# locuslab/icnn

Measured on NVIDIA H100. Metric: inner-loop solves/sec (batch x iters), higher is better.
Workload: dtype f32 (K1 PICNN f/grad) + f64 (K2 bundle solve)

## Files before the change

icnn_b200/csrc/bundle_pc.cu:

```cuda
#include "bundle_pc_kernel.cuh"

#include <cstdio>
#include <cstdlib>

namespace icnn {

#define ICNN_PC_DECL(NAME) cudaError_t launch_pc_##NAME(const PcArgs& a, const PcConfig& c, int B, cudaStream_t st)
ICNN_PC_DECL(1x1); ICNN_PC_DECL(1x2);
ICNN_PC_DECL(1x1_scalar); ICNN_PC_DECL(1x2_scalar);
ICNN_PC_DECL(8x2);
ICNN_PC_DECL(16x2); ICNN_PC_DECL(16x4);
ICNN_PC_DECL(v3_8x4);

ICNN_PC_DECL(1x1) { return launch_pc<1, 1, true>(a, c, B, st); }
ICNN_PC_DECL(1x2) { return launch_pc<1, 2, true>(a, c, B, st); }
ICNN_PC_DECL(1x1_scalar) { return launch_pc<1, 1, false>(a, c, B, st); }
ICNN_PC_DECL(1x2_scalar) { return launch_pc<1, 2, false>(a, c, B, st); }

struct PcTestEnv { bool v3, split5; int pfa, pfb; };
static PcTestEnv pc_test_env() {
  PcTestEnv e = {true, false, 1, 8};
  if (const char* v = getenv("ICNN_PC_V3")) e.v3 = v[0] != '0';
  if (const char* v = getenv("ICNN_PC_LEGACY")) e.split5 = v[0] == '1';
  if (const char* v = getenv("ICNN_PC_PREFETCH")) {
    int pa = 0, pb = 0;
    if (sscanf(v, "%d,%d", &pa, &pb) == 2 && pa >= 0 && pa <= 8 && pb >= 0 && pb <= 64) { e.pfa = pa; e.pfb = pb; }
  }
  return e;
}

static bool pc_fits(const icnn_bundle_bufs* b, int wps, int nch, bool v3, PcConfig* out) {
  if (b->n > 128 * wps * nch) return false;
  PcConfig c;
  c.wps = wps; c.nch = nch; c.v3 = v3;
  c.npad = (b->n + 15) & ~15;
  c.vec = (b->n & 3) == 0;
  if (!c.vec && wps > 1) return false;
  c.smem = sizeof(double) * pc_group_doubles(c.npad, b->KS, wps, v3);
  if (c.smem > 227 * 1024) return false;
  if (v3) {
    if (!c.vec || 2 * (c.smem + 1024) > 228 * 1024) return false;
    c.minb = 2;
  } else if (wps == 16) c.minb = 1;
  else if (wps == 1) c.minb = 2;
  else
    c.minb = (c.smem + 1024) * (24 / wps) <= 228 * 1024 ? 3 : 2;
  *out = c;
  return true;
}

static bool pick_pc(const icnn_bundle_bufs* b, bool allow_v3, PcConfig* out) {
  const int n = b->n;
  if (b->KS > 62) return false;
  if (n <= 128) return pc_fits(b, 1, 1, false, out);
  if (n <= 256) return pc_fits(b, 1, 2, false, out);
  if (n <= 1024) return false;
  if (n <= 2048) return pc_fits(b, 8, 2, false, out);
  if (n <= 4096) return (allow_v3 && pc_fits(b, 8, 4, true, out)) || pc_fits(b, 16, 2, false, out);
  return pc_fits(b, 16, 4, false, out);
}

int bundle_pc_launch(const icnn_bundle_cfg* cfg, const icnn_bundle_bufs* b, int t, cudaStream_t st) {
  const PcTestEnv env = pc_test_env();
  PcConfig c;
  if (!pick_pc(b, env.v3, &c)) return ICNN_E_UNSUPPORTED;
  PcArgs a;
  a.b = *b; a.c = *cfg; a.t = t; a.npad = c.npad;
  a.split5 = env.split5; a.pfa = env.pfa; a.pfb = env.pfb;
  cudaError_t e;
  if (c.v3) e = launch_pc_v3_8x4(a, c, b->B, st);
  else if (c.wps == 16) e = c.nch == 2 ? launch_pc_16x2(a, c, b->B, st) : launch_pc_16x4(a, c, b->B, st);
  else if (c.wps == 8) e = launch_pc_8x2(a, c, b->B, st);
  else if (c.vec) e = c.nch == 1 ? launch_pc_1x1(a, c, b->B, st) : launch_pc_1x2(a, c, b->B, st);
  else e = c.nch == 1 ? launch_pc_1x1_scalar(a, c, b->B, st) : launch_pc_1x2_scalar(a, c, b->B, st);
  if (e != cudaSuccess) {
    set_error("bundle_pc launch (wps=%d nch=%d v3=%d smem=%zu): %s", c.wps, c.nch, (int)c.v3, c.smem, cudaGetErrorString(e));
    return ICNN_E_CUDA;
  }
  return ICNN_OK;
}

}
```

icnn_b200/csrc/bundle_pc_kernel.cuh:

```cuda
#pragma once
#include "bundle_step_kernel.cuh"

namespace icnn {

struct PcArgs {
  icnn_bundle_bufs b;
  icnn_bundle_cfg c;
  int t;
  int npad;
  int pfa;
  int pfb;
  bool split5;
};

__device__ __forceinline__ void prefetch_l2(const void* p) { asm volatile("prefetch.global.L2 [%0];" ::"l"(p)); }

constexpr int PC_NKV = 18;
constexpr int PC_NKV_V3 = 12;

__host__ __device__ inline size_t pc_group_doubles(int npad, int KS, int wps, bool v3) {
  size_t d = (size_t)(v3 ? 3 : 4) * npad + (size_t)KS * (KS + 1) / 2 +
             (size_t)(v3 ? PC_NKV_V3 : PC_NKV) * KS + KS  +
             8 * wps  + 16  + 4 ;
  return (d + 1) & ~(size_t)1;
}

__device__ __forceinline__ int lidx(int r, int c) { return r * (r + 1) / 2 + c; }

__device__ __forceinline__ double chol_dot(const double* a, const double* b, int c) {
  double t0 = 0.0, t1 = 0.0, t2 = 0.0, t3 = 0.0;
  int p = 0;
  for (; p + 3 < c; p += 4) {
    t0 = fma(a[p], b[p], t0);
    t1 = fma(a[p + 1], b[p + 1], t1);
    t2 = fma(a[p + 2], b[p + 2], t2);
    t3 = fma(a[p + 3], b[p + 3], t3);
  }
  for (; p < c; ++p) t0 = fma(a[p], b[p], t0);
  return (t0 + t1) + (t2 + t3);
}
template <bool K32>
__device__ __forceinline__ bool warp_cholesky_impl(double* L, double* invd, int k, int lane) {
  bool ok = true;
  const int r0 = lane, r1 = lane + 32;
  const int o0 = lidx(r0, 0), o1 = lidx(r1, 0);
  for (int c = 0; c < k; ++c) {
    const int oc = lidx(c, 0);
    double s0 = 0.0, s1 = 0.0;
    if (r0 >= c && r0 < k) s0 = L[o0 + c] - chol_dot(L + o0, L + oc, c);
    if (!K32) { if (r1 >= c && r1 < k) s1 = L[o1 + c] - chol_dot(L + o1, L + oc, c); }
    const double piv = K32 ? __shfl_sync(0xffffffffu, s0, c) : __shfl_sync(0xffffffffu, (c < 32) ? s0 : s1, c & 31);
    if (!(piv > 0.0) || !isfinite(piv)) { ok = false; break; }
    const double inv = rsqrt(piv);
    if (r0 > c && r0 < k) L[o0 + c] = s0 * inv;
    if (!K32) { if (r1 > c && r1 < k) L[o1 + c] = s1 * inv; }
    if (lane == 0) { L[oc + c] = piv * inv; invd[c] = inv; }
    __syncwarp();
  }
  __syncwarp();
  return ok;
}
__device__ inline bool warp_cholesky_p(double* L, double* invd, int k, int lane) {
  return k <= 32 ? warp_cholesky_impl<true>(L, invd, k, lane) : warp_cholesky_impl<false>(L, invd, k, lane);
}

template <int NR, bool K32>
__device__ __forceinline__ void warp_chol_solve_impl(const double* L, const double* invd, int k, double (&b0)[NR],
                                                     double (&b1)[NR], int lane) {
  const int r0 = lane, r1 = lane + 32;
  const int o0 = lidx(r0, 0), o1 = lidx(r1, 0);
  for (int i = 0; i < k; ++i) {
    const double di = invd[i];
    const double l0 = (r0 > i && r0 < k) ? L[o0 + i] : 0.0;
    const double l1 = (!K32 && r1 > i && r1 < k) ? L[o1 + i] : 0.0;
#pragma unroll
    for (int q = 0; q < NR; ++q) {
      const double xi = (K32 ? __shfl_sync(0xffffffffu, b0[q], i) : __shfl_sync(0xffffffffu, (i < 32) ? b0[q] : b1[q], i & 31)) * di;
      b0[q] = (r0 == i) ? xi : fma(-l0, xi, b0[q]);
      if (!K32) b1[q] = (r1 == i) ? xi : fma(-l1, xi, b1[q]);
    }
  }
  for (int i = k - 1; i >= 0; --i) {
    const double di = invd[i];
    const int oi = lidx(i, 0);
    const double l0 = (r0 < i) ? L[oi + r0] : 0.0;
    const double l1 = (!K32 && r1 < i) ? L[oi + r1] : 0.0;
#pragma unroll
    for (int q = 0; q < NR; ++q) {
      const double xi = (K32 ? __shfl_sync(0xffffffffu, b0[q], i) : __shfl_sync(0xffffffffu, (i < 32) ? b0[q] : b1[q], i & 31)) * di;
      b0[q] = (r0 == i) ? xi : fma(-l0, xi, b0[q]);
      if (!K32) b1[q] = (r1 == i) ? xi : fma(-l1, xi, b1[q]);
    }
  }
}
template <int NR>
__device__ inline void warp_chol_solve_p(const double* L, const double* invd, int k, double (&b0)[NR],
                                         double (&b1)[NR], int lane) {
  if (k <= 32) warp_chol_solve_impl<NR, true>(L, invd, k, b0, b1, lane);
  else warp_chol_solve_impl<NR, false>(L, invd, k, b0, b1, lane);
}

__device__ __forceinline__ double step2(double v0, double d0, bool ok0, double v1, double d1, bool ok1) {
  double a = 1e300;
  bool any = false;
  if (ok0 && d0 < 0.0) { a = -v0 / d0; any = true; }
  if (ok1 && d1 < 0.0) { a = fmin(a, -v1 / d1); any = true; }
  a = Grp<1>::wmin(a);
  any = __any_sync(0xffffffffu, any);
  return any ? a : 1.0;
}

template <int WPS>
struct PcRed {
  double* red;
  int par;
  template <class G>
  __device__ __forceinline__ double sum(const G& g, double v) {
    v = Grp<WPS>::wsum(v);
    if (WPS == 1) { __syncwarp(); return v; }
    double* r = red + par * 4 * WPS;
    par ^= 1;
    if (g.lane == 0) r[g.warp] = v;
    g.sync();
    double a = 0.0;
#pragma unroll
    for (int w = 0; w < WPS; ++w) a += r[w];
    return a;
  }
  template <class G>
  __device__ __forceinline__ void min2(const G& g, double& a, double& b) {
    a = Grp<WPS>::wmin(a);
    b = Grp<WPS>::wmin(b);
    if (WPS == 1) { __syncwarp(); return; }
    double* r = red + par * 4 * WPS;
    par ^= 1;
    if (g.lane == 0) { r[g.warp] = a; r[WPS + g.warp] = b; }
    g.sync();
    double ra = r[0], rb = r[WPS];
#pragma unroll
    for (int w = 1; w < WPS; ++w) { ra = fmin(ra, r[w]); rb = fmin(rb, r[WPS + w]); }
    a = ra; b = rb;
  }
};

__device__ __forceinline__ double dweight(double y) { return fma(-y, y, y); }

template <int WPS, int NA, int NB, bool TRI, bool PSEUDO, bool VEC, class G>
__device__ __forceinline__ void gram_sweep_pc(const G& g, const float* const* rowp, int k, int n, const double* yv,
                                              const double* rv, double* Lp, double* qk, double* wk, double* scratch,
                                              int scap, int a0, int b0, int pfd = 0) {
  constexpr int NT = TRI ? NA * (NA + 1) / 2 : NA * NB;
  constexpr int NL = TRI ? NB : NA + NB;
  double acc[NT][2];
#pragma unroll
  for (int t = 0; t < NT; ++t) acc[t][0] = acc[t][1] = 0.0;
  const int r = g.lane >> 2, q = g.lane & 3;
  const float* rp[NL];
  bool rok[NL];
#pragma unroll
  for (int b = 0; b < NL; ++b) {
    const int blk = TRI ? (b0 + b) : (b < NA ? a0 + b : b0 + (b - NA));
    const int row = blk * 8 + r - 2;
    rok[b] = row >= 0 && row < k;
    rp[b] = rowp[rok[b] ? row : 0] + 4 * q;
  }
  const bool ps = PSEUDO && r < 2;
  const double* yq = yv + 4 * q;
  const double* rq = rv + 4 * q;
  const int ngrp = (n + 15) >> 4;
  constexpr int NG = (NT <= 6) ? 2 : 1;
#pragma unroll 1
  for (int gi = g.warp; gi < ngrp; gi += NG * WPS) {
    float4 v[NG][NL];
#pragma unroll
    for (int u = 0; u < NG; ++u) {
      const int gu = gi + u * WPS;
      const int off = gu * 16;
      const int col = off + 4 * q;
      const bool gv = (u == 0) || gu < ngrp;
#pragma unroll
      for (int b = 0; b < NL; ++b) {
        v[u][b] = make_float4(0.f, 0.f, 0.f, 0.f);
        if (VEC) {
          if (gv && rok[b] && col < n) v[u][b] = *reinterpret_cast<const float4*>(rp[b] + off);
        } else if (gv && rok[b]) {
          const float* p = rp[b] + off;
          if (col < n) v[u][b].x = p[0];
          if (col + 1 < n) v[u][b].y = p[1];
          if (col + 2 < n) v[u][b].z = p[2];
          if (col + 3 < n) v[u][b].w = p[3];
        }
      }
    }
    if (pfd > 0) {
#pragma unroll
      for (int u = 0; u < NG; ++u) {
        const int col = (gi + (pfd * NG + u) * WPS) * 16 + 4 * q;
        if (col < n) {
#pragma unroll
          for (int b = 0; b < NL; ++b) if (rok[b]) prefetch_l2(rp[b] + (col - 4 * q));
        }
      }
    }
#pragma unroll
    for (int u = 0; u < NG; ++u) {
      const int gu = gi + u * WPS;
      if (u > 0 && gu >= ngrp) break;
      const int off = gu * 16;
      const double2 ya = *reinterpret_cast<const double2*>(yq + off);
      const double2 yb = *reinterpret_cast<const double2*>(yq + off + 2);
      double dd[4] = {dweight(ya.x), dweight(ya.y), dweight(yb.x), dweight(yb.y)};
      double pa[4] = {0.0, 0.0, 0.0, 0.0};
      if (PSEUDO && ps) {
        if (r == 0) {
          const double2 ra = *reinterpret_cast<const double2*>(rq + off);
          const double2 rb = *reinterpret_cast<const double2*>(rq + off + 2);
          pa[0] = dd[0] * ra.x; pa[1] = dd[1] * ra.y; pa[2] = dd[2] * rb.x; pa[3] = dd[3] * rb.y;
        } else {
          pa[0] = ya.x; pa[1] = ya.y; pa[2] = yb.x; pa[3] = yb.y;
        }
      }
#pragma unroll
      for (int s = 0; s < 4; ++s) {
        double f[NL];
#pragma unroll
        for (int b = 0; b < NL; ++b)
          f[b] = (double)((s == 0) ? v[u][b].x : (s == 1) ? v[u][b].y : (s == 2) ? v[u][b].z : v[u][b].w);
        int t = 0;
#pragma unroll
        for (int i = 0; i < NA; ++i) {
          const double af = (PSEUDO && i == 0) ? fma(f[0], dd[s], pa[s]) : f[i] * dd[s];
#pragma unroll
          for (int j = TRI ? i : 0; j < NB; ++j) { dmma884(acc[t][0], acc[t][1], af, f[TRI ? j : NA + j]); ++t; }
        }
      }
    }
  }
  if (WPS > 1) {
    constexpr int SLAB = NT * 64;
    const int cap = scap / SLAB;
    g.sync();
    if (cap >= 1) {
      int active = WPS;
      while (active > 1) {
        const int m = ::min(cap, active >> 1);
        if (g.warp >= active - m && g.warp < active) {
          double* sl = scratch + (size_t)(g.warp - (active - m)) * SLAB + g.lane;
#pragma unroll
          for (int t = 0; t < NT; ++t) { sl[(2 * t) * 32] = acc[t][0]; sl[(2 * t + 1) * 32] = acc[t][1]; }
        }
        g.sync();
        if (g.warp >= active - 2 * m && g.warp < active - m) {
          const double* sl = scratch + (size_t)(g.warp - (active - 2 * m)) * SLAB + g.lane;
#pragma unroll
          for (int t = 0; t < NT; ++t) { acc[t][0] += sl[(2 * t) * 32]; acc[t][1] += sl[(2 * t + 1) * 32]; }
        }
        active -= m;
        if (active > 1) g.sync();
      }
    } else {
      for (int wi = 1; wi < WPS; ++wi) {
        if (g.warp == wi) {
          int t = 0;
#pragma unroll
          for (int i = 0; i < NA; ++i)
#pragma unroll
            for (int j = TRI ? i : 0; j < NB; ++j) {
#pragma unroll
              for (int h = 0; h < 2; ++h) {
                const int ii = (a0 + i) * 8 + r, jj = (b0 + j) * 8 + 2 * q + h;
                if (jj >= 2 && jj < k + 2) {
                  if (ii < 2) { if (PSEUDO && i == 0) { double* d = (ii == 0 ? qk : wk) + (jj - 2); *d = (wi == 1 ? 0.0 : *d) + acc[t][h]; } }
                  else if (ii < k + 2 && (!(TRI && i == j) || jj >= ii)) { double* d = Lp + lidx(jj - 2, ii - 2); *d = (wi == 1 ? 0.0 : *d) + acc[t][h]; }
                }
              }
              ++t;
            }
        }
        g.sync();
      }
    }
  }
  if (g.warp == 0) {
    const bool addin = (WPS > 1) && (scap / (NT * 64) < 1);
    int t = 0;
#pragma unroll
    for (int i = 0; i < NA; ++i)
#pragma unroll
      for (int j = TRI ? i : 0; j < NB; ++j) {
#pragma unroll
        for (int h = 0; h < 2; ++h) {
          const int ii = (a0 + i) * 8 + r, jj = (b0 + j) * 8 + 2 * q + h;
          if (jj >= 2 && jj < k + 2) {
            if (ii < 2) {
              if (PSEUDO && i == 0) { double* d = (ii == 0 ? qk : wk) + (jj - 2); *d = (addin ? *d : 0.0) + acc[t][h]; }
            } else if (ii < k + 2 && (!(TRI && i == j) || jj >= ii)) {
              double* d = Lp + lidx(jj - 2, ii - 2);
              *d = (addin ? *d : 0.0) + acc[t][h];
            }
          }
        }
        ++t;
      }
    __syncwarp();
  }
}

template <int WPS, int NB, bool VEC, class G>
__device__ __forceinline__ void gram_rect_pair_pc(const G& g, const float* const* rowp, int k, int n, const double* yv,
                                                  const double* rv, double* Lp, double* qk, double* wk, double* sx, int scap,
                                                  int pfd) {
  gram_sweep_pc<WPS, 2, NB, false, true, VEC>(g, rowp, k, n, yv, rv, Lp, qk, wk, sx, scap, 0, 4, pfd);
  gram_sweep_pc<WPS, 2, NB, false, false, VEC>(g, rowp, k, n, yv, rv, Lp, qk, wk, sx, scap, 2, 4, pfd);
}

template <int WPS, bool VEC, bool ONE5, class G>
__device__ __forceinline__ void gram_pass_pc(const G& g, const float* const* rowp, int k, int n, const double* yv,
                                             const double* rv, double* Lp, double* qk, double* wk, double* sx, int scap,
                                             bool split5, int pfd) {
  const int rb = (k + 2 + 7) >> 3;
  if (rb == 1) gram_sweep_pc<WPS, 1, 1, true, true, VEC>(g, rowp, k, n, yv, rv, Lp, qk, wk, sx, scap, 0, 0, pfd);
  else if (rb == 2) gram_sweep_pc<WPS, 2, 2, true, true, VEC>(g, rowp, k, n, yv, rv, Lp, qk, wk, sx, scap, 0, 0, pfd);
  else if (rb == 3) gram_sweep_pc<WPS, 3, 3, true, true, VEC>(g, rowp, k, n, yv, rv, Lp, qk, wk, sx, scap, 0, 0, pfd);
  else if (ONE5 && rb == 5 && !split5) {
    if constexpr (ONE5) gram_sweep_pc<WPS, 5, 5, true, true, VEC>(g, rowp, k, n, yv, rv, Lp, qk, wk, sx, scap, 0, 0, pfd);
  } else {
    gram_sweep_pc<WPS, 4, 4, true, true, VEC>(g, rowp, k, n, yv, rv, Lp, qk, wk, sx, scap, 0, 0, pfd);
    if (rb > 4) {
      const int r2 = rb - 4;
      if (r2 == 1) { gram_sweep_pc<WPS, 1, 1, true, false, VEC>(g, rowp, k, n, yv, rv, Lp, qk, wk, sx, scap, 4, 4, pfd); gram_rect_pair_pc<WPS, 1, VEC>(g, rowp, k, n, yv, rv, Lp, qk, wk, sx, scap, pfd); }
      else if (r2 == 2) { gram_sweep_pc<WPS, 2, 2, true, false, VEC>(g, rowp, k, n, yv, rv, Lp, qk, wk, sx, scap, 4, 4, pfd); gram_rect_pair_pc<WPS, 2, VEC>(g, rowp, k, n, yv, rv, Lp, qk, wk, sx, scap, pfd); }
      else if (r2 == 3) { gram_sweep_pc<WPS, 3, 3, true, false, VEC>(g, rowp, k, n, yv, rv, Lp, qk, wk, sx, scap, 4, 4, pfd); gram_rect_pair_pc<WPS, 3, VEC>(g, rowp, k, n, yv, rv, Lp, qk, wk, sx, scap, pfd); }
      else { gram_sweep_pc<WPS, 4, 4, true, false, VEC>(g, rowp, k, n, yv, rv, Lp, qk, wk, sx, scap, 4, 4, pfd); gram_rect_pair_pc<WPS, 4, VEC>(g, rowp, k, n, yv, rv, Lp, qk, wk, sx, scap, pfd); }
    }
  }
}

template <int T, bool VEC>
__device__ __forceinline__ int pc_col(int cb, int tid, int c) { return VEC ? cb + 4 * tid + c : cb + tid + c * T; }

template <int T, int NR, bool VEC, int UNR = 4>
__device__ __forceinline__ void col_dots_pc(const float* const* rowp, int k, int n, int cb, int tid,
                                            const double* const (&w)[NR], double (&acc)[NR][4], int pfr = 0) {
#pragma unroll
  for (int q = 0; q < NR; ++q)
#pragma unroll
    for (int c = 0; c < 4; ++c) acc[q][c] = 0.0;
  const bool in0 = VEC ? (cb + 4 * tid < n) : (cb + tid < n);
  const bool full = VEC ? in0 : (cb + tid + 3 * T < n);
#pragma unroll UNR
  for (int j = 0; j < k; ++j) {
    const float* p = rowp[j];
    float v[4] = {0.f, 0.f, 0.f, 0.f};
    if (VEC && pfr > 0 && in0) {
      const int jp = j + pfr;
      if (jp < k) prefetch_l2(rowp[jp] + cb + 4 * tid);
      else if (jp - k < k && cb + 4 * T + 4 * tid < n) prefetch_l2(rowp[jp - k] + cb + 4 * T + 4 * tid);
    }
    if (VEC) {
      if (in0) { const float4 x = *reinterpret_cast<const float4*>(p + cb + 4 * tid); v[0] = x.x; v[1] = x.y; v[2] = x.z; v[3] = x.w; }
    } else {
#pragma unroll
      for (int c = 0; c < 4; ++c) if (full || cb + tid + c * T < n) v[c] = p[cb + tid + c * T];
    }
#pragma unroll
    for (int q = 0; q < NR; ++q) {
      const double wq = w[q][j];
#pragma unroll
      for (int c = 0; c < 4; ++c) acc[q][c] = fma((double)v[c], wq, acc[q][c]);
    }
  }
}

__device__ __forceinline__ void ratio_min(double& nm, double& dn, double a, double b) {
  if (a * dn < nm * b) { nm = a; dn = b; }
}

struct PcKxk {
  double* Lp; double* invd; const double* zc; const double* scur; const double* wk; const double* hk; const double* qk;
  double* dza; double* dzp; double* dzq; double* dsa; double* sc; int* isc;
};
template <bool K32>
__device__ __forceinline__ void pc_kxk_stage(const PcKxk& io, int k, int lane, double pr) {
  double* Lp = io.Lp;
  const int j0 = lane, j1 = lane + 32;
  const bool v0 = j0 < k, v1ok = !K32 && j1 < k;
  const double tt = io.sc[0];
  const double z0 = v0 ? io.zc[j0] : 0.0, z1 = v1ok ? io.zc[j1] : 0.0;
  const double s0 = v0 ? io.scur[j0] : 0.0, s1 = v1ok ? io.scur[j1] : 0.0;
  const double rd0 = v0 ? ((io.wk[j0] + io.hk[j0]) - tt) + s0 : 0.0;
  const double rd1 = v1ok ? ((io.wk[j1] + io.hk[j1]) - tt) + s1 : 0.0;
  const double zs = Grp<1>::wsum(z0 + z1);
  const double dr = Grp<1>::wsum(fma(rd0, rd0, rd1 * rd1));
  const double rt = 1.0 - zs;
  const bool conv = (sqrt(pr + rt * rt) < 1e-8 && sqrt(dr) < 1e-8);
  if (conv) {
    if (lane == 0) io.isc[2] = 1;
  } else {
    if (v0) Lp[lidx(j0, j0)] += s0 / z0;
    if (v1ok) Lp[lidx(j1, j1)] += s1 / z1;
    __syncwarp();
    const bool ok = warp_cholesky_impl<K32>(Lp, io.invd, k, lane);
    if (!ok) { if (lane == 0) io.isc[3] = 1; }
    else {
      const double mu = Grp<1>::wsum(fma(s0, z0, s1 * z1)) / k;
      const double ra0 = v0 ? rd0 - io.qk[j0] - s0 : 0.0, ra1 = v1ok ? rd1 - io.qk[j1] - s1 : 0.0;
      const double rp0 = v0 ? mu / z0 : 0.0, rp1 = v1ok ? mu / z1 : 0.0;
      double b0[3] = {v0 ? 1.0 : 0.0, ra0, rp0}, b1[3] = {v1ok ? 1.0 : 0.0, ra1, rp1};
      warp_chol_solve_impl<3, K32>(Lp, io.invd, k, b0, b1, lane);
      const double w1s = Grp<1>::wsum(b0[0] + b1[0]);
      const double dta = (Grp<1>::wsum(fma(ra0, b0[0], ra1 * b1[0])) - rt) / w1s;
      const double dtp = Grp<1>::wsum(fma(rp0, b0[0], rp1 * b1[0])) / w1s;
      const double da0 = fma(-dta, b0[0], b0[1]), da1 = fma(-dta, b1[0], b1[1]);
      const double dp0 = fma(-dtp, b0[0], b0[2]), dp1 = fma(-dtp, b1[0], b1[2]);
      const double dsa0 = v0 ? -(s0 / z0) * (z0 + da0) : 0.0, dsa1 = v1ok ? -(s1 / z1) * (z1 + da1) : 0.0;
      const double rq0 = v0 ? -(dsa0 * da0) / z0 : 0.0, rq1 = v1ok ? -(dsa1 * da1) / z1 : 0.0;
      double c0[1] = {rq0}, c1[1] = {rq1};
      warp_chol_solve_impl<1, K32>(Lp, io.invd, k, c0, c1, lane);
      const double dtq = Grp<1>::wsum(fma(rq0, b0[0], rq1 * b1[0])) / w1s;
      if (v0) { io.dza[j0] = da0; io.dzp[j0] = dp0; io.dzq[j0] = fma(-dtq, b0[0], c0[0]); io.dsa[j0] = dsa0; }
      if (v1ok) { io.dza[j1] = da1; io.dzp[j1] = dp1; io.dzq[j1] = fma(-dtq, b1[0], c1[0]); io.dsa[j1] = dsa1; }
      if (lane == 0) { io.sc[1] = dta; io.sc[2] = dtp; io.sc[3] = dtq; }
    }
  }
  __syncwarp();
}

template <int WPS, int NCH, bool R80, bool VEC, bool V3>
__global__ void __launch_bounds__(WPS * 32, WPS == 16 ? 1 : (R80 ? 24 : 16) / WPS) bundle_pc_kernel(PcArgs A) {
  const icnn_bundle_bufs& b = A.b;
  const icnn_bundle_cfg& cf = A.c;
  if (b.nactive[A.t] == 0) return;
  extern __shared__ __align__(16) double smem_d[];
  constexpr int GPB = 1;
  constexpr int T = WPS * 32;
  static_assert(NCH == 1 || NCH == 2 || NCH == 4, "NCH");
  Grp<WPS> g;
  g.tid = threadIdx.x % T;
  g.lane = threadIdx.x & 31;
  g.warp = g.tid >> 5;
  g.gid = threadIdx.x / T;
  const int u = blockIdx.x * GPB + g.gid;
  if (u >= b.B) return;
  if (b.finished[u]) return;

  const int n = b.n, KS = b.KS, npad = A.npad;
  double* base = smem_d + (size_t)g.gid * pc_group_doubles(npad, KS, WPS, V3);
  double* yv = base;
  double* uv = V3 ? nullptr : yv + npad;
  double* rv = V3 ? yv + npad : uv + npad;
  double* xv = rv + npad;
  double* Lp = xv + npad;
  double* kv = Lp + (size_t)KS * (KS + 1) / 2;
#define PCKV(i) (kv + (i) * KS)
  double* hk = PCKV(0);
  double* wk = PCKV(5);
  double* qk = PCKV(6);
  double* dza = PCKV(7);
  double* dzp = PCKV(8);
  double* dzq = PCKV(9);
  double* dsa = PCKV(10);
  double* invd = PCKV(11);
  double* tk = PCKV(V3 ? 7 : 12);
  double* ek = PCKV(V3 ? 8 : 13);
  double* rk = PCKV(V3 ? 9 : 14);
  const float** rowp = reinterpret_cast<const float**>(kv + (size_t)(V3 ? PC_NKV_V3 : PC_NKV) * KS);
  PcRed<WPS> red;
  red.red = reinterpret_cast<double*>(rowp + KS);
  red.par = 0;
  g.red = red.red;
  double* sc = red.red + 8 * WPS;
  int* isc = reinterpret_cast<int*>(sc + 16);

  const int k0 = b.count[u];
  const int k = k0 + 1;
  const int* permu = b.perm + (size_t)u * KS;
  float* Gu = b.G + (size_t)u * KS * n;
  double* hu = b.h + (size_t)u * KS;
  double* lamu = b.lam + (size_t)u * KS;
  double* rsu = b.rsum + (size_t)u * KS;
  double* gramu = b.gram + (size_t)u * KS * KS;
  double* yu = b.y + (size_t)u * n;
  const int slot_new = permu[k0];

  for (int j = g.tid; j < k; j += T) rowp[j] = Gu + (size_t)permu[j] * n;
  if (g.tid == 0) {
#pragma unroll
    for (int i = 0; i < 8; ++i) isc[i] = 0;
  }
  g.sync();
  const float* gnew = rowp[k0];

  {
    double hs = 0.0, rs = 0.0, bad = 0.0, ent = 0.0;
    double* ysrow = b.ys ? b.ys + ((size_t)u * KS + slot_new) * n : nullptr;
    for (int e = g.tid; e < n; e += T) {
      const double ge = (double)gnew[e];
      const double ye = yu[e];
      hs = fma(ge, ye, hs);
      rs += ge;
      if (!isfinite(ge)) bad = 1.0;
      if (ysrow) __stcs(ysrow + e, ye);
      if (b.iter_stats) ent += neg_entropy(ye);
    }
    if (b.iter_stats) ent = g.sum(ent);
    hs = g.sum(hs);
    rs = g.sum(rs);
    bad = g.max(bad);
    const double fu = b.f64 ? b.f64[u] : (double)b.f[u];
    if (g.tid == 0) { stat_add(b.iter_stats, A.t, 0, 1.0); stat_add(b.iter_stats, A.t, 6, fu + ent); }
    if (bad > 0.0 || !isfinite(fu)) {
      if (g.tid == 0) { b.status[u] = ICNN_ST_NONFINITE; b.finished[u] = 1; b.nIters[u] = A.t - 1; stat_add(b.iter_stats, A.t, 5, 1.0); }
      return;
    }
    for (int j = g.warp; j < k; j += WPS) {
      const float* rj = rowp[j];
      double acc = 0.0;
      int diff = 0;
      for (int e = g.lane; e < n; e += 32) {
        const float a = rj[e], c = gnew[e];
        acc = fma((double)a, (double)c, acc);
        diff |= (a != c);
      }
      acc = Grp<WPS>::wsum(acc);
      diff = __any_sync(0xffffffffu, diff);
      if (g.lane == 0) { tk[j] = acc; ek[j] = diff ? 1.0 : 0.0; }
    }
    if (g.tid == 0) { hu[slot_new] = fu - hs; rsu[slot_new] = rs; sc[10] = fu - hs; sc[11] = rs; }
    g.sync();
    if (g.tid == 0) {
      int dup = 0;
      for (int j = 0; j < k0; ++j) dup |= (ek[j] == 0.0);
      isc[0] = dup;
    }
    g.sync();
  }
  bool dependent = false;
  if (k > n) dependent = true;
  else if (k0 > 0) {
    if (g.warp == 0) {
      for (int i = g.lane; i < k0; i += 32)
        for (int j = 0; j <= i; ++j) Lp[lidx(i, j)] = gramu[(size_t)permu[i] * KS + permu[j]];
      __syncwarp();
      const bool ok = warp_cholesky_p(Lp, invd, k0, g.lane);
      if (ok) {
        double b0[1] = {g.lane < k0 ? tk[g.lane] : 0.0}, b1[1] = {g.lane + 32 < k0 ? tk[g.lane + 32] : 0.0};
        warp_chol_solve_p<1>(Lp, invd, k0, b0, b1, g.lane);
        if (g.lane < k0) rk[g.lane] = b0[0];
        if (g.lane + 32 < k0) rk[g.lane + 32] = b1[0];
      }
      double md = tk[k0];
      for (int j = g.lane; j < k0; j += 32) md = fmax(md, gramu[(size_t)permu[j] * KS + permu[j]]);
      md = Grp<1>::wmax(md);
      if (g.lane == 0) { isc[1] = ok ? 1 : 0; sc[9] = md; }
      __syncwarp();
    }
    g.sync();
    const double maxdiag = sc[9];
    if (isc[0]) dependent = true;
    else if (!isc[1]) dependent = false;
    else {
      const double thr2 = cf.rank_tol * cf.rank_tol * maxdiag;
      for (int rep = 0; rep < 2; ++rep) {
        double p = 0.0;
        col_pass<T>(rowp, k0, n, g.tid, rk, [&](int e, double a) {
          const double r = (rep ? xv[e] : (double)gnew[e]) - a;
          xv[e] = r;
          p = fma(r, r, p);
        });
        p = g.sum(p);
        if (p <= thr2) { dependent = true; break; }
        if (rep == 1 || p > 1e-8 * maxdiag) break;
        g.sync();
        for (int j = g.warp; j < k0; j += WPS) {
          double acc = 0.0;
          for (int e = g.lane; e < n; e += 32) acc = fma((double)rowp[j][e], xv[e], acc);
          acc = Grp<WPS>::wsum(acc);
          if (g.lane == 0) rk[j] = acc;
        }
        g.sync();
        if (g.warp == 0) {
          double b0[1] = {g.lane < k0 ? rk[g.lane] : 0.0}, b1[1] = {g.lane + 32 < k0 ? rk[g.lane + 32] : 0.0};
          warp_chol_solve_p<1>(Lp, invd, k0, b0, b1, g.lane);
          if (g.lane < k0) rk[g.lane] = b0[0];
          if (g.lane + 32 < k0) rk[g.lane + 32] = b1[0];
        }
        g.sync();
      }
    }
  } else {
    dependent = !(tk[0] > 0.0);
  }
  if (dependent) {
    if (g.tid == 0) { b.status[u] = ICNN_ST_RANK_STOP; b.finished[u] = 1; b.nIters[u] = A.t - 1; stat_add(b.iter_stats, A.t, 5, 1.0); }
    return;
  }
  for (int j = g.tid; j < k; j += T) {
    gramu[(size_t)slot_new * KS + permu[j]] = tk[j];
    gramu[(size_t)permu[j] * KS + slot_new] = tk[j];
    hk[j] = (j == k0) ? sc[10] : hu[permu[j]];
    PCKV(1)[j] = 1.0 / k;
    PCKV(3)[j] = 1.0;
  }
  if (g.tid == 0) sc[0] = 1.0;
  for (int e = n + g.tid; e < npad; e += T) { yv[e] = 0.5; rv[e] = 0.0; }
  g.sync();

  const int maxit = cf.max_inner > 0 ? cf.max_inner : 20;
  int inner_its = 0, fail = 0;
  int zsel = 0;
  double pr = 0.0;
  {
    const double* const w1r[1] = {PCKV(1)};
#pragma unroll 1
    for (int ch = 0; ch < NCH; ++ch) {
      const int cb = ch * 4 * T;
      if (cb >= n) break;
      double acc[1][4];
      col_dots_pc<T, 1, VEC>(rowp, k, n, cb, g.tid, w1r, acc);
#pragma unroll
      for (int c = 0; c < 4; ++c) {
        const int e = pc_col<T, VEC>(cb, g.tid, c);
        if (e < n) { yv[e] = 0.5; if (!V3) uv[e] = acc[0][c]; rv[e] = acc[0][c]; pr = fma(acc[0][c], acc[0][c], pr); }
      }
    }
  }
  pr = red.sum(g, pr);
  const int j0 = g.lane, j1 = g.lane + 32;
  const bool v0 = j0 < k, v1ok = j1 < k;
#pragma unroll 1
  for (int it = 0; it < maxit; ++it) {
    double* zc = PCKV(1 + zsel);
    double* scur = PCKV(3 + zsel);
    gram_pass_pc<WPS, VEC, V3>(g, rowp, k, n, yv, rv, Lp, qk, wk, xv, npad, A.split5, V3 ? A.pfa : 0);
    if (g.warp == 0) {
      const PcKxk io{Lp, invd, zc, scur, wk, hk, qk, dza, dzp, dzq, dsa, sc, isc};
      if (k <= 32) pc_kxk_stage<true>(io, k, g.lane, pr);
      else pc_kxk_stage<false>(io, k, g.lane, pr);
    }
    g.sync();
    if (isc[2]) break;
    if (isc[3]) { fail = 1; break; }
    inner_its = it + 1;
    double x2a[4], x2b[4], x2c[4], x2d[4];
    double n1 = 1.0, d1 = 0.0, n2 = 1.0, d2 = 0.0;
    {
      const double* const w3[3] = {dza, dzp, dzq};
#pragma unroll 1
      for (int ch = 0; ch < NCH; ++ch) {
        const int cb = ch * 4 * T;
        if (cb >= n) break;
        double acc[3][4];
        col_dots_pc<T, 3, VEC, V3 ? 8 : 4>(rowp, k, n, cb, g.tid, w3, acc, V3 ? A.pfb : 0);
#pragma unroll
        for (int c = 0; c < 4; ++c) {
          const int e = pc_col<T, VEC>(cb, g.tid, c);
          if (e < n) {
            const double ye = yv[e];
            const double dy = -dweight(ye) * (rv[e] + acc[0][c]);
            if (dy < 0.0) ratio_min(n1, d1, ye, -dy);
            if (dy > 0.0) ratio_min(n2, d2, 1.0 - ye, dy);
            xv[e] = acc[0][c] + acc[2][c];
          }
          const double v2 = acc[1][c];
          if (ch == 0) x2a[c] = v2; else if (ch == 1) x2b[c] = v2; else if (ch == 2) x2c[c] = v2; else x2d[c] = v2;
        }
      }
    }
    double st = d1 > 0.0 ? n1 / d1 : 1e300, st2 = d2 > 0.0 ? n2 / d2 : 1e300;
    red.min2(g, st, st2);
    st = fmin(st > 1e299 ? 1.0 : st, st2 > 1e299 ? 1.0 : st2);
    const double z0 = v0 ? zc[j0] : 0.0, z1 = v1ok ? zc[j1] : 0.0;
    const double s0 = v0 ? scur[j0] : 0.0, s1 = v1ok ? scur[j1] : 0.0;
    const double da0 = v0 ? dza[j0] : 0.0, da1 = v1ok ? dza[j1] : 0.0;
    const double dsa0 = v0 ? dsa[j0] : 0.0, dsa1 = v1ok ? dsa[j1] : 0.0;
    double dz0, dz1, ds0, ds1, dtt, sig;
    {
      const double alpha = fmin(fmin(step2(z0, da0, v0, z1, da1, v1ok), step2(s0, dsa0, v0, s1, dsa1, v1ok)), fmin(st, 1.0));
      const double num = Grp<1>::wsum(fma(s0 + alpha * dsa0, z0 + alpha * da0, (s1 + alpha * dsa1) * (z1 + alpha * da1)));
      const double den = Grp<1>::wsum(fma(s0, z0, s1 * z1));
      const double sg = num / den;
      sig = sg * sg * sg;
      const double mu = den / k;
      const double dzc0 = v0 ? fma(sig, dzp[j0], dzq[j0]) : 0.0, dzc1 = v1ok ? fma(sig, dzp[j1], dzq[j1]) : 0.0;
      const double rc0 = v0 ? -(mu * sig - dsa0 * da0) / s0 : 0.0, rc1 = v1ok ? -(mu * sig - dsa1 * da1) / s1 : 0.0;
      dz0 = da0 + dzc0; dz1 = da1 + dzc1;
      ds0 = v0 ? dsa0 - (s0 / z0) * (rc0 + dzc0) : 0.0;
      ds1 = v1ok ? dsa1 - (s1 / z1) * (rc1 + dzc1) : 0.0;
      dtt = sc[1] + fma(sig, sc[2], sc[3]);
    }
    n1 = 1.0; d1 = 0.0; n2 = 1.0; d2 = 0.0;
#pragma unroll 1
    for (int ch = 0; ch < NCH; ++ch) {
      const int cb = ch * 4 * T;
      if (cb >= n) break;
#pragma unroll
      for (int c = 0; c < 4; ++c) {
        const int e = pc_col<T, VEC>(cb, g.tid, c);
        const double v2 = (ch == 0) ? x2a[c] : (ch == 1) ? x2b[c] : (ch == 2) ? x2c[c] : x2d[c];
        if (e < n) {
          const double ye = yv[e];
          const double du = fma(sig, v2, xv[e]);
          const double dy = -dweight(ye) * (rv[e] + du);
          if (dy < 0.0) ratio_min(n1, d1, ye, -dy);
          if (dy > 0.0) ratio_min(n2, d2, 1.0 - ye, dy);
          if (V3) xv[e] = du;
          else { xv[e] = dy; rv[e] = du; }
        }
      }
    }
    st = d1 > 0.0 ? n1 / d1 : 1e300; st2 = d2 > 0.0 ? n2 / d2 : 1e300;
    red.min2(g, st, st2);
    st = fmin(st > 1e299 ? 1.0 : st, st2 > 1e299 ? 1.0 : st2);
    double a = fmin(fmin(step2(s0, ds0, v0, s1, ds1, v1ok), step2(z0, dz0, v0, z1, dz1, v1ok)), st);
    a = fmax(0.0, fmin(1.0, 0.99 * a));
    if (g.warp == 0) {
      double* zn = PCKV(2 - zsel);
      double* snew = PCKV(4 - zsel);
      if (v0) { zn[j0] = fma(a, dz0, z0); snew[j0] = fma(a, ds0, s0); }
      if (v1ok) { zn[j1] = fma(a, dz1, z1); snew[j1] = fma(a, ds1, s1); }
      if (g.lane == 0) sc[0] += a * dtt;
    }
    zsel ^= 1;
    pr = 0.0;
#pragma unroll 1
    for (int ch = 0; ch < NCH; ++ch) {
      const int cb = ch * 4 * T;
      if (cb >= n) break;
#pragma unroll (WPS == 1 ? 1 : 4)
      for (int c = 0; c < 4; ++c) {
        const int e = pc_col<T, VEC>(cb, g.tid, c);
        if (e < n) {
          if (V3) {
            const double yo = yv[e], ro = rv[e], du = xv[e];
            const double dy = -dweight(yo) * (ro + du);
            const double uo = ro - log(yo / (1.0 - yo));
            const double ye = fma(a, dy, yo);
            const double ue = fma(a, du, uo);
            const double r = log(ye / (1.0 - ye)) + ue;
            yv[e] = ye; rv[e] = r;
            pr = fma(r, r, pr);
          } else {
            const double ye = fma(a, xv[e], yv[e]);
            const double ue = fma(a, rv[e], uv[e]);
            const double r = log(ye / (1.0 - ye)) + ue;
            yv[e] = ye; uv[e] = ue; rv[e] = r;
            pr = fma(r, r, pr);
          }
        }
      }
    }
    pr = red.sum(g, pr);
  }
  g.sync();
  const double* zfin = PCKV(1 + zsel);

  double bad = 0.0;
  for (int e = g.tid; e < n; e += T) {
    const double ye = yv[e];
    if (!isfinite(ye)) bad = 1.0;
    yu[e] = ye;
    b.y32[(size_t)u * n + e] = (float)ye;
  }
  bad = g.max(bad);
  if (g.tid == 0) {
    int nk = 0, nd = 0;
    int* oldp = reinterpret_cast<int*>(tk);
    int* dropped = oldp + KS;
    int* pw = b.perm + (size_t)u * KS;
    for (int j = 0; j < k; ++j) oldp[j] = pw[j];
    for (int j = 0; j < k; ++j) {
      const double lj = zfin[j];
      if (lj > cf.prune_thr) { pw[nk++] = oldp[j]; lamu[oldp[j]] = lj; }
      else dropped[nd++] = oldp[j];
    }
    for (int j = 0; j < nd; ++j) pw[nk + j] = dropped[j];
    b.count[u] = nk;
    int fin = 0;
    int stt = ICNN_ST_RUNNING;
    if (fail || b.status[u] == ICNN_ST_SOLVE_FAIL) stt = ICNN_ST_SOLVE_FAIL;
    if (bad > 0.0) { stt = ICNN_ST_NONFINITE; fin = 1; }
    b.status[u] = stt;
    if (fin) b.finished[u] = 1;
    else atomicAdd(&b.nactive[A.t + 1], 1);
    if (b.newton_its) b.newton_its[u] += inner_its;
    if (b.ksum) b.ksum[u] += k;
    if (b.iter_stats) {
      stat_add(b.iter_stats, A.t, 1, (double)k);
      stat_add(b.iter_stats, A.t, 2, (double)inner_its);
      stat_add(b.iter_stats, A.t, 3, (double)inner_its * k * k);
      stat_add(b.iter_stats, A.t, 4, (double)inner_its * k);
      if (fin) stat_add(b.iter_stats, A.t, 5, 1.0);
    }
  }
#undef PCKV
}

struct PcConfig { int wps, nch, npad, minb; bool vec, v3; size_t smem; };

template <int WPS, int NCH, bool VEC, bool V3 = false>
static cudaError_t launch_pc(const PcArgs& a, const PcConfig& c, int B, cudaStream_t st) {
  void (*kern)(PcArgs);
  if constexpr (V3 || WPS == 16 || WPS == 1) kern = bundle_pc_kernel<WPS, NCH, false, VEC, V3>;
  else kern = (c.minb >= 3) ? bundle_pc_kernel<WPS, NCH, true, VEC, false> : bundle_pc_kernel<WPS, NCH, false, VEC, false>;
  cudaError_t e = cudaFuncSetAttribute(kern, cudaFuncAttributeMaxDynamicSharedMemorySize, (int)c.smem);
  if (e != cudaSuccess) return e;
  if constexpr (V3) {
    e = cudaFuncSetAttribute(kern, cudaFuncAttributePreferredSharedMemoryCarveout, cudaSharedmemCarveoutMaxShared);
    if (e != cudaSuccess) return e;
  }
  kern<<<(unsigned)B, WPS * 32, c.smem, st>>>(a);
  return cudaGetLastError();
}

}
```

Measured before the change: 190,500.

## Add block-parallel tiled Cholesky KxK stage using DMMA for multi-warp PC kernels

Replaces the single-warp KxK Cholesky factor-and-solve stage with a blocked 8x8-tile version for kernels with more than one warp per group. Trailing tile updates run on FP64 tensor-core mma (dmma884) and are spread across all warps. The tiles live in the xv scratch buffer. The goal is to shorten the serial per-iteration KxK stage, at the cost of extra block syncs and padding K up to multiples of 8. It is on by default and can be disabled through an environment variable.

```diff
diff --git a/icnn_b200/csrc/bundle_pc.cu b/icnn_b200/csrc/bundle_pc.cu
--- a/icnn_b200/csrc/bundle_pc.cu
+++ b/icnn_b200/csrc/bundle_pc.cu
@@ -2,6 +2,7 @@
 
 #include <cstdio>
 #include <cstdlib>
+#include <cstring>
 
 namespace icnn {
 
@@ -17,11 +18,12 @@
 ICNN_PC_DECL(1x1_scalar) { return launch_pc<1, 1, false>(a, c, B, st); }
 ICNN_PC_DECL(1x2_scalar) { return launch_pc<1, 2, false>(a, c, B, st); }
 
-struct PcTestEnv { bool v3, split5; int pfa, pfb; };
+struct PcTestEnv { bool v3, split5, kxk; int pfa, pfb; };
 static PcTestEnv pc_test_env() {
-  PcTestEnv e = {true, false, 1, 8};
+  PcTestEnv e = {true, false, true, 1, 8};
   if (const char* v = getenv("ICNN_PC_V3")) e.v3 = v[0] != '0';
   if (const char* v = getenv("ICNN_PC_LEGACY")) e.split5 = v[0] == '1';
+  if (const char* v = getenv("ICNN_PC_KXK")) e.kxk = strcmp(v, "warp") != 0;
   if (const char* v = getenv("ICNN_PC_PREFETCH")) {
     int pa = 0, pb = 0;
     if (sscanf(v, "%d,%d", &pa, &pb) == 2 && pa >= 0 && pa <= 8 && pb >= 0 && pb <= 64) { e.pfa = pa; e.pfb = pb; }
@@ -29,12 +31,13 @@
   return e;
 }
 
-static bool pc_fits(const icnn_bundle_bufs* b, int wps, int nch, bool v3, PcConfig* out) {
+static bool pc_fits(const icnn_bundle_bufs* b, int wps, int nch, bool v3, bool kxk, PcConfig* out) {
   if (b->n > 128 * wps * nch) return false;
   PcConfig c;
   c.wps = wps; c.nch = nch; c.v3 = v3;
   c.npad = (b->n + 15) & ~15;
   c.vec = (b->n & 3) == 0;
+  c.kxk = kxk && wps > 1 && pc_kxk_tile_doubles(b->KS) <= (size_t)c.npad;
   if (!c.vec && wps > 1) return false;
   c.smem = sizeof(double) * pc_group_doubles(c.npad, b->KS, wps, v3);
   if (c.smem > 227 * 1024) return false;
@@ -49,24 +52,25 @@
   return true;
 }
 
-static bool pick_pc(const icnn_bundle_bufs* b, bool allow_v3, PcConfig* out) {
+static bool pick_pc(const icnn_bundle_bufs* b, const PcTestEnv& env, PcConfig* out) {
   const int n = b->n;
+  const bool kx = env.kxk;
   if (b->KS > 62) return false;
-  if (n <= 128) return pc_fits(b, 1, 1, false, out);
-  if (n <= 256) return pc_fits(b, 1, 2, false, out);
+  if (n <= 128) return pc_fits(b, 1, 1, false, kx, out);
+  if (n <= 256) return pc_fits(b, 1, 2, false, kx, out);
   if (n <= 1024) return false;
-  if (n <= 2048) return pc_fits(b, 8, 2, false, out);
-  if (n <= 4096) return (allow_v3 && pc_fits(b, 8, 4, true, out)) || pc_fits(b, 16, 2, false, out);
-  return pc_fits(b, 16, 4, false, out);
+  if (n <= 2048) return pc_fits(b, 8, 2, false, kx, out);
+  if (n <= 4096) return (env.v3 && pc_fits(b, 8, 4, true, kx, out)) || pc_fits(b, 16, 2, false, kx, out);
+  return pc_fits(b, 16, 4, false, kx, out);
 }
 
 int bundle_pc_launch(const icnn_bundle_cfg* cfg, const icnn_bundle_bufs* b, int t, cudaStream_t st) {
   const PcTestEnv env = pc_test_env();
   PcConfig c;
-  if (!pick_pc(b, env.v3, &c)) return ICNN_E_UNSUPPORTED;
+  if (!pick_pc(b, env, &c)) return ICNN_E_UNSUPPORTED;
   PcArgs a;
   a.b = *b; a.c = *cfg; a.t = t; a.npad = c.npad;
-  a.split5 = env.split5; a.pfa = env.pfa; a.pfb = env.pfb;
+  a.split5 = env.split5; a.pfa = env.pfa; a.pfb = env.pfb; a.kxk = c.kxk;
   cudaError_t e;
   if (c.v3) e = launch_pc_v3_8x4(a, c, b->B, st);
   else if (c.wps == 16) e = c.nch == 2 ? launch_pc_16x2(a, c, b->B, st) : launch_pc_16x4(a, c, b->B, st);
diff --git a/icnn_b200/csrc/bundle_pc_kernel.cuh b/icnn_b200/csrc/bundle_pc_kernel.cuh
--- a/icnn_b200/csrc/bundle_pc_kernel.cuh
+++ b/icnn_b200/csrc/bundle_pc_kernel.cuh
@@ -11,6 +11,7 @@
   int pfa;
   int pfb;
   bool split5;
+  bool kxk;
 };
 
 __device__ __forceinline__ void prefetch_l2(const void* p) { asm volatile("prefetch.global.L2 [%0];" ::"l"(p)); }
@@ -426,6 +427,194 @@
   __syncwarp();
 }
 
+__host__ __device__ inline size_t pc_kxk_tile_doubles(int KS) {
+  const int nb = (KS + 7) >> 3;
+  return (size_t)64 * (nb * (nb + 1) / 2 + nb) + 8 * nb;
+}
+__device__ __forceinline__ int ktile(int I, int J) { return (I * (I + 1) / 2 + J) * 64; }
+
+template <bool FWD>
+__device__ __forceinline__ void kxk_tile_solve(const double* kt, const double* invd, double* R, int nb, int lane) {
+  const int r = lane >> 2, q = lane & 3;
+  for (int s = 0; s < nb; ++s) {
+    const int J = FWD ? s : nb - 1 - s;
+    const double* L = kt + ktile(J, J);
+    double* RJ = R + J * 64;
+    if (lane < 8) {
+      double x[8];
+#pragma unroll
+      for (int i = 0; i < 8; ++i) x[i] = RJ[i * 8 + lane];
+#pragma unroll
+      for (int ii = 0; ii < 8; ++ii) {
+        const int i = FWD ? ii : 7 - ii;
+        x[i] *= invd[J * 8 + i];
+#pragma unroll
+        for (int j = 0; j < 8; ++j)
+          if (FWD ? j > i : j < i) x[j] = fma(-(FWD ? L[j * 8 + i] : L[i * 8 + j]), x[i], x[j]);
+      }
+#pragma unroll
+      for (int i = 0; i < 8; ++i) RJ[i * 8 + lane] = x[i];
+    }
+    __syncwarp();
+    for (int I = FWD ? J + 1 : 0; I < (FWD ? nb : J); ++I) {
+      double* RI = R + I * 64;
+      double d0 = RI[r * 8 + 2 * q], d1 = RI[r * 8 + 2 * q + 1];
+#pragma unroll
+      for (int kk = 0; kk < 2; ++kk) {
+        const double a = FWD ? kt[ktile(I, J) + r * 8 + 4 * kk + q] : kt[ktile(J, I) + (4 * kk + q) * 8 + r];
+        dmma884(d0, d1, -a, RJ[(4 * kk + q) * 8 + r]);
+      }
+      RI[r * 8 + 2 * q] = d0; RI[r * 8 + 2 * q + 1] = d1;
+    }
+    __syncwarp();
+  }
+}
+__device__ __forceinline__ void kxk_tile_chol_solve(const double* kt, const double* invd, double* R, int nb, int lane) {
+  kxk_tile_solve<true>(kt, invd, R, nb, lane);
+  kxk_tile_solve<false>(kt, invd, R, nb, lane);
+}
+
+template <int WPS, class G>
+__device__ __forceinline__ void pc_kxk_blocked(const G& g, const PcKxk& io, double* kt, int k, double pr) {
+  g.sync();
+  const int lane = g.lane;
+  const int j0 = lane, j1 = lane + 32;
+  const bool v0 = j0 < k, v1ok = j1 < k;
+  const double tt = io.sc[0];
+  const double z0 = v0 ? io.zc[j0] : 0.0, z1 = v1ok ? io.zc[j1] : 0.0;
+  const double s0 = v0 ? io.scur[j0] : 0.0, s1 = v1ok ? io.scur[j1] : 0.0;
+  const double rd0 = v0 ? ((io.wk[j0] + io.hk[j0]) - tt) + s0 : 0.0;
+  const double rd1 = v1ok ? ((io.wk[j1] + io.hk[j1]) - tt) + s1 : 0.0;
+  const double zs = Grp<1>::wsum(z0 + z1);
+  const double dr = Grp<1>::wsum(fma(rd0, rd0, rd1 * rd1));
+  const double rt = 1.0 - zs;
+  if (sqrt(pr + rt * rt) < 1e-8 && sqrt(dr) < 1e-8) {
+    if (g.warp == 0 && lane == 0) io.isc[2] = 1;
+    return;
+  }
+  const int nb = (k + 7) >> 3;
+  const int ntile = nb * (nb + 1) / 2;
+  for (int e = g.tid; e < ntile * 64; e += WPS * 32) {
+    int I = 0;
+    while ((I + 1) * (I + 2) / 2 * 64 <= e) ++I;
+    const int J = e / 64 - I * (I + 1) / 2;
+    const int row = I * 8 + ((e >> 3) & 7), col = J * 8 + (e & 7);
+    double v = (row == col) ? 1.0 : 0.0;
+    if (row < k && col < k) {
+      v = io.Lp[row >= col ? lidx(row, col) : lidx(col, row)];
+      if (row == col) v += io.scur[row] / io.zc[row];
+    }
+    kt[e] = v;
+  }
+  g.sync();
+  double* R = kt + ntile * 64;
+  double* tinv = R + nb * 64;
+  const int r = lane >> 2, q = lane & 3;
+  for (int J = 0; J < nb; ++J) {
+    if (g.warp == 0) {
+      double* T = kt + ktile(J, J);
+      double a[8];
+#pragma unroll
+      for (int j = 0; j < 8; ++j) a[j] = lane < 8 ? T[(lane & 7) * 8 + j] : 0.0;
+      bool ok = true;
+      double myinv = 0.0;
+#pragma unroll
+      for (int c = 0; c < 8; ++c) {
+        const double piv = __shfl_sync(0xffffffffu, a[c], c);
+        if (!(piv > 0.0) || !isfinite(piv)) { ok = false; break; }
+        const double inv = rsqrt(piv);
+        const double l = (lane > c) ? a[c] * inv : 0.0;
+        if (lane == c) { a[c] = piv * inv; myinv = inv; }
+        else if (lane > c) a[c] = l;
+#pragma unroll
+        for (int j = c + 1; j < 8; ++j) {
+          const double lj = __shfl_sync(0xffffffffu, l, j);
+          if (lane >= j) a[j] = fma(-l, lj, a[j]);
+        }
+      }
+      if (!ok) { if (lane == 0) io.isc[3] = 1; }
+      else if (lane < 8) {
+#pragma unroll
+        for (int j = 0; j < 8; ++j) T[lane * 8 + j] = a[j];
+        tinv[J * 8 + lane] = myinv;
+      }
+    }
+    g.sync();
+    if (io.isc[3]) return;
+    if (J + 1 == nb) break;
+    for (int I = J + 1 + g.warp; I < nb; I += WPS) {
+      if (lane < 8) {
+        const double* L = kt + ktile(J, J);
+        double* P = kt + ktile(I, J);
+        double x[8];
+#pragma unroll
+        for (int c = 0; c < 8; ++c) x[c] = P[lane * 8 + c];
+#pragma unroll
+        for (int c = 0; c < 8; ++c) {
+          x[c] *= tinv[J * 8 + c];
+#pragma unroll
+          for (int j = c + 1; j < 8; ++j) x[j] = fma(-x[c], L[j * 8 + c], x[j]);
+        }
+#pragma unroll
+        for (int c = 0; c < 8; ++c) P[lane * 8 + c] = x[c];
+      }
+    }
+    g.sync();
+    const int m = nb - 1 - J;
+    for (int t = g.warp; t < m * (m + 1) / 2; t += WPS) {
+      int ii = 0;
+      while ((ii + 1) * (ii + 2) / 2 <= t) ++ii;
+      const int I = J + 1 + ii, K = J + 1 + (t - ii * (ii + 1) / 2);
+      double* D = kt + ktile(I, K);
+      const double* LI = kt + ktile(I, J);
+      const double* LK = kt + ktile(K, J);
+      double d0 = D[r * 8 + 2 * q], d1 = D[r * 8 + 2 * q + 1];
+#pragma unroll
+      for (int kk = 0; kk < 2; ++kk) dmma884(d0, d1, -LI[r * 8 + 4 * kk + q], LK[r * 8 + 4 * kk + q]);
+      D[r * 8 + 2 * q] = d0; D[r * 8 + 2 * q + 1] = d1;
+    }
+    g.sync();
+  }
+  if (g.warp != 0) return;
+  const double mu = Grp<1>::wsum(fma(s0, z0, s1 * z1)) / k;
+  const double ra0 = v0 ? rd0 - io.qk[j0] - s0 : 0.0, ra1 = v1ok ? rd1 - io.qk[j1] - s1 : 0.0;
+  const double rp0 = v0 ? mu / z0 : 0.0, rp1 = v1ok ? mu / z1 : 0.0;
+  const bool w0 = j0 < nb * 8, w1 = j1 < nb * 8;
+  double* R0 = R + (j0 >> 3) * 64 + (j0 & 7) * 8;
+  double* R1 = R + (j1 >> 3) * 64 + (j1 & 7) * 8;
+#pragma unroll
+  for (int c = 0; c < 8; ++c) {
+    if (w0) R0[c] = c == 0 ? (v0 ? 1.0 : 0.0) : c == 1 ? ra0 : c == 2 ? rp0 : 0.0;
+    if (w1) R1[c] = c == 0 ? (v1ok ? 1.0 : 0.0) : c == 1 ? ra1 : c == 2 ? rp1 : 0.0;
+  }
+  __syncwarp();
+  kxk_tile_chol_solve(kt, tinv, R, nb, lane);
+  double b0[3], b1[3];
+#pragma unroll
+  for (int c = 0; c < 3; ++c) { b0[c] = v0 ? R0[c] : 0.0; b1[c] = v1ok ? R1[c] : 0.0; }
+  const double w1s = Grp<1>::wsum(b0[0] + b1[0]);
+  const double dta = (Grp<1>::wsum(fma(ra0, b0[0], ra1 * b1[0])) - rt) / w1s;
+  const double dtp = Grp<1>::wsum(fma(rp0, b0[0], rp1 * b1[0])) / w1s;
+  const double da0 = fma(-dta, b0[0], b0[1]), da1 = fma(-dta, b1[0], b1[1]);
+  const double dp0 = fma(-dtp, b0[0], b0[2]), dp1 = fma(-dtp, b1[0], b1[2]);
+  const double dsa0 = v0 ? -(s0 / z0) * (z0 + da0) : 0.0, dsa1 = v1ok ? -(s1 / z1) * (z1 + da1) : 0.0;
+  const double rq0 = v0 ? -(dsa0 * da0) / z0 : 0.0, rq1 = v1ok ? -(dsa1 * da1) / z1 : 0.0;
+  __syncwarp();
+#pragma unroll
+  for (int c = 0; c < 8; ++c) {
+    if (w0) R0[c] = c == 0 ? rq0 : 0.0;
+    if (w1) R1[c] = c == 0 ? rq1 : 0.0;
+  }
+  __syncwarp();
+  kxk_tile_chol_solve(kt, tinv, R, nb, lane);
+  const double c0 = v0 ? R0[0] : 0.0, c1 = v1ok ? R1[0] : 0.0;
+  const double dtq = Grp<1>::wsum(fma(rq0, b0[0], rq1 * b1[0])) / w1s;
+  if (v0) { io.dza[j0] = da0; io.dzp[j0] = dp0; io.dzq[j0] = fma(-dtq, b0[0], c0); io.dsa[j0] = dsa0; }
+  if (v1ok) { io.dza[j1] = da1; io.dzp[j1] = dp1; io.dzq[j1] = fma(-dtq, b1[0], c1); io.dsa[j1] = dsa1; }
+  if (lane == 0) { io.sc[1] = dta; io.sc[2] = dtp; io.sc[3] = dtq; }
+  __syncwarp();
+}
+
 template <int WPS, int NCH, bool R80, bool VEC, bool V3>
 __global__ void __launch_bounds__(WPS * 32, WPS == 16 ? 1 : (R80 ? 24 : 16) / WPS) bundle_pc_kernel(PcArgs A) {
   const icnn_bundle_bufs& b = A.b;
@@ -633,10 +822,13 @@
     double* zc = PCKV(1 + zsel);
     double* scur = PCKV(3 + zsel);
     gram_pass_pc<WPS, VEC, V3>(g, rowp, k, n, yv, rv, Lp, qk, wk, xv, npad, A.split5, V3 ? A.pfa : 0);
-    if (g.warp == 0) {
+    {
       const PcKxk io{Lp, invd, zc, scur, wk, hk, qk, dza, dzp, dzq, dsa, sc, isc};
-      if (k <= 32) pc_kxk_stage<true>(io, k, g.lane, pr);
-      else pc_kxk_stage<false>(io, k, g.lane, pr);
+      if (WPS > 1 && A.kxk) pc_kxk_blocked<WPS>(g, io, xv, k, pr);
+      else if (g.warp == 0) {
+        if (k <= 32) pc_kxk_stage<true>(io, k, g.lane, pr);
+        else pc_kxk_stage<false>(io, k, g.lane, pr);
+      }
     }
     g.sync();
     if (isc[2]) break;
@@ -796,7 +988,7 @@
 #undef PCKV
 }
 
-struct PcConfig { int wps, nch, npad, minb; bool vec, v3; size_t smem; };
+struct PcConfig { int wps, nch, npad, minb; bool vec, v3, kxk; size_t smem; };
 
 template <int WPS, int NCH, bool VEC, bool V3 = false>
 static cudaError_t launch_pc(const PcArgs& a, const PcConfig& c, int B, cudaStream_t st) {
```

After: 194,200, median of 6. 2.0% higher.
